# cloneofsimo/paint-with-words-sd

Hardware: NVIDIA H100
Metric: unet_steps_per_sec_512sq_cfg (higher is better)
Workload: dtype f16

## Files before the change

paint_with_words_sd_b200/csrc/attn_tc.cuh:

```cuda
#pragma once
#include "mma_sm90.cuh"
#include "pww_common.cuh"
#include "xattn_core.cuh"
#include "xattn_tc.cuh"

namespace pww {
namespace fa {

constexpr int kThreads = core::kThreads;
constexpr int kBM = core::kBM;
constexpr int kBN = 64;

template <int D>
struct Cfg {
  using T_ = core::Tile<D>;
  static constexpr uint32_t KVBYTES = kBN * T_::LD * 2;
  static constexpr uint32_t OFF_KV = T_::QBYTES;
  static constexpr uint32_t SMEM = T_::QBYTES + 2 * 2 * KVBYTES;
  static_assert(SMEM <= 232448, "shared memory budget");
};

struct Params {
  const __half* q;
  const __half* k;
  const __half* v;
  __half* out;
  int B, H, N;
  int64_t bs, rs;
  int64_t o_bs, o_rs;
  float scale;
};

template <int D>
__global__ void __launch_bounds__(kThreads) attn_fwd_kernel(const Params p) {
  using C = core::Tile<D>;
  using CF = Cfg<D>;
  extern __shared__ __align__(128) unsigned char smem[];
  const uint32_t smem0 = ptx::smem_u32(smem);
  const int warp = threadIdx.x >> 5, lane = threadIdx.x & 31;
  const int qtiles = (p.N + kBM - 1) / kBM;
  const int bh = blockIdx.x / qtiles, qt = blockIdx.x - bh * qtiles;
  const int b = bh / p.H, h = bh - b * p.H;
  const int row_base = qt * kBM;
  const __half* qb = p.q + (int64_t)b * p.bs + h * D;
  const __half* kb = p.k + (int64_t)b * p.bs + h * D;
  const __half* vb = p.v + (int64_t)b * p.bs + h * D;
  const int ntiles = (p.N + kBN - 1) / kBN;
  auto issue_kv = [&](int j) {
    const uint32_t st = smem0 + CF::OFF_KV + (j & 1) * 2 * CF::KVBYTES;
    const int rows = p.N - j * kBN < kBN ? p.N - j * kBN : kBN;
    core::load_rows<D>(st, kb + (int64_t)j * kBN * p.rs, p.rs, kBN, rows);
    core::load_rows<D>(st + CF::KVBYTES, vb + (int64_t)j * kBN * p.rs, p.rs, kBN, rows);
    ptx::cp_async_commit();
  };
  {
    const int rows = p.N - row_base < kBM ? p.N - row_base : kBM;
    core::load_rows<D>(smem0, qb + (int64_t)row_base * p.rs, p.rs, kBM, rows);
  }
  issue_kv(0);
  uint32_t qa[C::KS][4];
  float o[C::NT][4];
#pragma unroll
  for (int j = 0; j < C::NT; ++j) o[j][0] = o[j][1] = o[j][2] = o[j][3] = 0.f;
  float m0 = -INFINITY, m1 = -INFINITY, l0 = 0.f, l1 = 0.f;
  const float sl2 = p.scale * 1.4426950408889634f;
  const uint32_t qs = smem0 + (uint32_t)(warp * 16 * C::LD) * 2u;
#pragma unroll 1
  for (int jt = 0; jt < ntiles; ++jt) {
    if (jt + 1 < ntiles) {
      issue_kv(jt + 1);
      ptx::cp_async_wait<1>();
    } else {
      ptx::cp_async_wait<0>();
    }
    __syncthreads();
    if (jt == 0) {
#pragma unroll
      for (int kk = 0; kk < C::KS; ++kk)
        ptx::ldsm_x4(qs + (uint32_t)((lane & 15) * C::LD + kk * 16 + (lane >> 4) * 8) * 2u, qa[kk][0], qa[kk][1], qa[kk][2], qa[kk][3]);
    }
    const uint32_t ks = smem0 + CF::OFF_KV + (jt & 1) * 2 * CF::KVBYTES, vs = ks + CF::KVBYTES;
    float s[8][4];
#pragma unroll
    for (int j = 0; j < 8; ++j) s[j][0] = s[j][1] = s[j][2] = s[j][3] = 0.f;
#pragma unroll
    for (int kk = 0; kk < C::KS; ++kk) {
#pragma unroll
      for (int jp = 0; jp < 4; ++jp) {
        const int t = 16 * jp + (lane & 7) + ((lane >> 4) << 3), d = kk * 16 + ((lane >> 3) & 1) * 8;
        uint32_t b0, b1, b2, b3;
        ptx::ldsm_x4(ks + (uint32_t)(t * C::LD + d) * 2u, b0, b1, b2, b3);
        ptx::mma16816(s[2 * jp], qa[kk], b0, b1);
        ptx::mma16816(s[2 * jp + 1], qa[kk], b2, b3);
      }
    }
    const int valid = p.N - jt * kBN;
    float t0 = -INFINITY, t1 = -INFINITY;
#pragma unroll
    for (int j = 0; j < 8; ++j)
#pragma unroll
      for (int e = 0; e < 4; ++e) {
        if (core::tok(j, e, lane) >= valid) s[j][e] = -INFINITY;
        if (e < 2) t0 = fmaxf(t0, s[j][e]); else t1 = fmaxf(t1, s[j][e]);
      }
    t0 = fmaxf(t0, __shfl_xor_sync(0xffffffffu, t0, 1));
    t0 = fmaxf(t0, __shfl_xor_sync(0xffffffffu, t0, 2));
    t1 = fmaxf(t1, __shfl_xor_sync(0xffffffffu, t1, 1));
    t1 = fmaxf(t1, __shfl_xor_sync(0xffffffffu, t1, 2));
    const float mn0 = fmaxf(m0, t0), mn1 = fmaxf(m1, t1);
    const float a0 = ptx::ex2((m0 - mn0) * sl2), a1 = ptx::ex2((m1 - mn1) * sl2);
    m0 = mn0; m1 = mn1;
    const float n0 = -mn0 * sl2, n1 = -mn1 * sl2;
    uint32_t pa[4][4];
    float r0 = 0.f, r1 = 0.f;
#pragma unroll
    for (int j = 0; j < 8; ++j) {
      const uint32_t p01 = ptx::pack_h2(ptx::ex2(fmaf(s[j][0], sl2, n0)), ptx::ex2(fmaf(s[j][1], sl2, n0)));
      const uint32_t p23 = ptx::pack_h2(ptx::ex2(fmaf(s[j][2], sl2, n1)), ptx::ex2(fmaf(s[j][3], sl2, n1)));
      const float2 f01 = ptx::unpack_h2(p01), f23 = ptx::unpack_h2(p23);
      r0 += f01.x + f01.y;
      r1 += f23.x + f23.y;
      pa[j >> 1][(j & 1) * 2] = p01;
      pa[j >> 1][(j & 1) * 2 + 1] = p23;
    }
    l0 = l0 * a0 + r0;
    l1 = l1 * a1 + r1;
#pragma unroll
    for (int j = 0; j < C::NT; ++j) {
      o[j][0] *= a0; o[j][1] *= a0; o[j][2] *= a1; o[j][3] *= a1;
    }
#pragma unroll
    for (int kk = 0; kk < 4; ++kk) {
      const int t = 16 * kk + (lane & 7) + ((lane >> 3) & 1) * 8;
#pragma unroll
      for (int jp = 0; jp < C::NT / 2; ++jp) {
        uint32_t b0, b1, b2, b3;
        ptx::ldsm_x4_t(vs + (uint32_t)(t * C::LD + 16 * jp + (lane >> 4) * 8) * 2u, b0, b1, b2, b3);
        ptx::mma16816(o[2 * jp], pa[kk], b0, b1);
        ptx::mma16816(o[2 * jp + 1], pa[kk], b2, b3);
      }
      if constexpr (C::NT & 1) {
        uint32_t b0, b1;
        ptx::ldsm_x2_t(vs + (uint32_t)(t * C::LD + 8 * (C::NT - 1)) * 2u, b0, b1);
        ptx::mma16816(o[C::NT - 1], pa[kk], b0, b1);
      }
    }
    __syncthreads();
  }
  l0 += __shfl_xor_sync(0xffffffffu, l0, 1);
  l0 += __shfl_xor_sync(0xffffffffu, l0, 2);
  l1 += __shfl_xor_sync(0xffffffffu, l1, 1);
  l1 += __shfl_xor_sync(0xffffffffu, l1, 2);
  const float i0 = 1.f / l0, i1 = 1.f / l1;
#pragma unroll
  for (int j = 0; j < C::NT; ++j) {
    o[j][0] *= i0; o[j][1] *= i0; o[j][2] *= i1; o[j][3] *= i1;
  }
  core::warp_store<D>(o, smem + warp * 16 * C::LD * 2, lane, p.out + (int64_t)b * p.o_bs + h * D, p.o_rs,
                      row_base + warp * 16, p.N);
}

template <int D>
cudaError_t launch(const void* q, const void* k, const void* v, void* out, int B, int H, int N, int64_t bs, int64_t rs,
                   int64_t o_bs, int64_t o_rs, float scale, cudaStream_t s) {
  using CF = Cfg<D>;
  Params p;
  p.q = (const __half*)q; p.k = (const __half*)k; p.v = (const __half*)v; p.out = (__half*)out;
  p.B = B; p.H = H; p.N = N; p.bs = bs; p.rs = rs; p.o_bs = o_bs; p.o_rs = o_rs; p.scale = scale;
  static bool attr_set[tc::kMaxDevices] = {false};
  if (!attr_set[tc::cur_device()]) {
    cudaError_t e = cudaFuncSetAttribute(attn_fwd_kernel<D>, cudaFuncAttributeMaxDynamicSharedMemorySize, CF::SMEM);
    if (e != cudaSuccess) return e;
    attr_set[tc::cur_device()] = true;
  }
  const long long grid = (long long)B * H * ((N + kBM - 1) / kBM);
  if (grid > 0x7fffffffLL) return cudaErrorInvalidConfiguration;
  attn_fwd_kernel<D><<<(unsigned)grid, kThreads, CF::SMEM, s>>>(p);
  return cudaGetLastError();
}

}
}
```

paint_with_words_sd_b200/csrc/mma_sm90.cuh:

```cuda
#pragma once
#include <cuda_fp16.h>
#include <cuda_runtime.h>
#include <stdint.h>

namespace pww {
namespace ptx {

__device__ __forceinline__ uint32_t smem_u32(const void* p) { return (uint32_t)__cvta_generic_to_shared(p); }

__device__ __forceinline__ void cp_async16(uint32_t dst, const void* src, uint32_t src_bytes) {
  asm volatile("cp.async.cg.shared.global [%0], [%1], 16, %2;" ::"r"(dst), "l"(src), "r"(src_bytes) : "memory");
}
__device__ __forceinline__ void cp_async_commit() { asm volatile("cp.async.commit_group;" ::: "memory"); }
template <int N>
__device__ __forceinline__ void cp_async_wait() { asm volatile("cp.async.wait_group %0;" ::"n"(N) : "memory"); }

__device__ __forceinline__ void ldsm_x4(uint32_t addr, uint32_t& r0, uint32_t& r1, uint32_t& r2, uint32_t& r3) {
  asm volatile("ldmatrix.sync.aligned.m8n8.x4.shared.b16 {%0, %1, %2, %3}, [%4];"
               : "=r"(r0), "=r"(r1), "=r"(r2), "=r"(r3) : "r"(addr));
}
__device__ __forceinline__ void ldsm_x4_t(uint32_t addr, uint32_t& r0, uint32_t& r1, uint32_t& r2, uint32_t& r3) {
  asm volatile("ldmatrix.sync.aligned.m8n8.x4.trans.shared.b16 {%0, %1, %2, %3}, [%4];"
               : "=r"(r0), "=r"(r1), "=r"(r2), "=r"(r3) : "r"(addr));
}
__device__ __forceinline__ void ldsm_x2_t(uint32_t addr, uint32_t& r0, uint32_t& r1) {
  asm volatile("ldmatrix.sync.aligned.m8n8.x2.trans.shared.b16 {%0, %1}, [%2];" : "=r"(r0), "=r"(r1) : "r"(addr));
}

__device__ __forceinline__ void mma16816(float* c, const uint32_t* a, uint32_t b0, uint32_t b1) {
  asm volatile(
      "mma.sync.aligned.m16n8k16.row.col.f32.f16.f16.f32 {%0, %1, %2, %3}, {%4, %5, %6, %7}, {%8, %9}, "
      "{%0, %1, %2, %3};"
      : "+f"(c[0]), "+f"(c[1]), "+f"(c[2]), "+f"(c[3])
      : "r"(a[0]), "r"(a[1]), "r"(a[2]), "r"(a[3]), "r"(b0), "r"(b1));
}

__device__ __forceinline__ float ex2(float x) {
  float y;
  asm("ex2.approx.ftz.f32 %0, %1;" : "=f"(y) : "f"(x));
  return y;
}
__device__ __forceinline__ uint32_t pack_h2(float lo, float hi) {
  const __half2 h = __floats2half2_rn(lo, hi);
  return *reinterpret_cast<const uint32_t*>(&h);
}
__device__ __forceinline__ float2 unpack_h2(uint32_t v) { return __half22float2(*reinterpret_cast<const __half2*>(&v)); }
__device__ __forceinline__ unsigned long long ld_acquire_gpu_u64(const unsigned long long* p) {
  unsigned long long v;
  asm volatile("ld.acquire.gpu.global.u64 %0, [%1];" : "=l"(v) : "l"(p) : "memory");
  return v;
}

}
}
```

Before: 145.0.

## Rewrite self-attention kernel as warp-specialized TMA plus WGMMA pipeline

Replaces the cp.async and mma.sync flash-attention kernel with a Hopper-style design. A producer warp issues TMA loads of Q/K/V into 128B-swizzled shared memory through a three-stage mbarrier ring. Two consumer warpgroups run QK^T and PV as asynchronous wgmma, interleaving the next tile's QK with the previous tile's PV behind ping-pong named barriers. Row sums come from an extra wgmma against a ones matrix rather than shuffles. It targets tensor-core throughput and load latency, at the cost of much more complex synchronization, one CTA per SM, and host-side tensor map encoding on every launch.

```diff
diff --git a/paint_with_words_sd_b200/csrc/attn_tc.cuh b/paint_with_words_sd_b200/csrc/attn_tc.cuh
--- a/paint_with_words_sd_b200/csrc/attn_tc.cuh
+++ b/paint_with_words_sd_b200/csrc/attn_tc.cuh
@@ -1,163 +1,269 @@
 #pragma once
+#include <cudaTypedefs.h>
+
 #include "mma_sm90.cuh"
 #include "pww_common.cuh"
-#include "xattn_core.cuh"
 #include "xattn_tc.cuh"
 
 namespace pww {
 namespace fa {
 
-constexpr int kThreads = core::kThreads;
-constexpr int kBM = core::kBM;
-constexpr int kBN = 64;
+constexpr int kWgRows = 64;
+constexpr int kConsumerWarps = 8;
+constexpr int kThreads = (kConsumerWarps + 1) * 32;
+constexpr int kBM = 2 * kWgRows;
 
 template <int D>
 struct Cfg {
-  using T_ = core::Tile<D>;
-  static constexpr uint32_t KVBYTES = kBN * T_::LD * 2;
-  static constexpr uint32_t OFF_KV = T_::QBYTES;
-  static constexpr uint32_t SMEM = T_::QBYTES + 2 * 2 * KVBYTES;
-  static_assert(SMEM <= 232448, "shared memory budget");
+  static_assert(D == 40 || D == 64 || D == 80 || D == 160, "head dims of SD1.5 (40 / 80 / 160) and SD2.x (64)");
+  static constexpr int SLABS = (D + 63) / 64;
+  static constexpr int KS = (D + 15) / 16;
+  static constexpr int NT = D / 8;
+  static constexpr int BN = D == 160 ? 64 : 128;
+  static constexpr int STAGES = 3;
+  static constexpr uint32_t QBYTES = kWgRows * SLABS * 128;
+  static constexpr uint32_t KVBYTES = BN * SLABS * 128;
+  static constexpr uint32_t OFF_KV = 2 * QBYTES;
+  static constexpr uint32_t OFF_ONES = OFF_KV + STAGES * 2 * KVBYTES;
+  static constexpr uint32_t OFF_BAR = OFF_ONES + 1024;
+  static constexpr uint32_t SMEM = OFF_BAR + (1 + 2 * STAGES) * 8 + 1024;
+  static_assert(SMEM <= 232448, "shared memory budget (227 KiB per CTA)");
 };
 
 struct Params {
-  const __half* q;
-  const __half* k;
-  const __half* v;
+  CUtensorMap tq, tk, tv;
   __half* out;
-  int B, H, N;
-  int64_t bs, rs;
+  int H, N;
+  int bmul;
   int64_t o_bs, o_rs;
   float scale;
 };
 
 template <int D>
-__global__ void __launch_bounds__(kThreads) attn_fwd_kernel(const Params p) {
-  using C = core::Tile<D>;
-  using CF = Cfg<D>;
-  extern __shared__ __align__(128) unsigned char smem[];
-  const uint32_t smem0 = ptx::smem_u32(smem);
-  const int warp = threadIdx.x >> 5, lane = threadIdx.x & 31;
+__global__ void __launch_bounds__(kThreads, 1) attn_fwd_kernel(const __grid_constant__ Params p) {
+  using C = Cfg<D>;
+  extern __shared__ unsigned char smem_raw[];
+  const uint32_t smem0 = (ptx::smem_u32(smem_raw) + 1023u) & ~1023u;
+  const uint32_t bar_q = smem0 + C::OFF_BAR, bar_full = bar_q + 8, bar_empty = bar_full + 8 * C::STAGES;
+  const int warp = __shfl_sync(0xffffffffu, threadIdx.x >> 5, 0), lane = threadIdx.x & 31;
   const int qtiles = (p.N + kBM - 1) / kBM;
   const int bh = blockIdx.x / qtiles, qt = blockIdx.x - bh * qtiles;
   const int b = bh / p.H, h = bh - b * p.H;
   const int row_base = qt * kBM;
-  const __half* qb = p.q + (int64_t)b * p.bs + h * D;
-  const __half* kb = p.k + (int64_t)b * p.bs + h * D;
-  const __half* vb = p.v + (int64_t)b * p.bs + h * D;
-  const int ntiles = (p.N + kBN - 1) / kBN;
-  auto issue_kv = [&](int j) {
-    const uint32_t st = smem0 + CF::OFF_KV + (j & 1) * 2 * CF::KVBYTES;
-    const int rows = p.N - j * kBN < kBN ? p.N - j * kBN : kBN;
-    core::load_rows<D>(st, kb + (int64_t)j * kBN * p.rs, p.rs, kBN, rows);
-    core::load_rows<D>(st + CF::KVBYTES, vb + (int64_t)j * kBN * p.rs, p.rs, kBN, rows);
-    ptx::cp_async_commit();
-  };
-  {
-    const int rows = p.N - row_base < kBM ? p.N - row_base : kBM;
-    core::load_rows<D>(smem0, qb + (int64_t)row_base * p.rs, p.rs, kBM, rows);
-  }
-  issue_kv(0);
-  uint32_t qa[C::KS][4];
+  const int ntiles = (p.N + C::BN - 1) / C::BN;
+  for (int i = threadIdx.x; i < 1024 / 16; i += blockDim.x)
+    *reinterpret_cast<uint4*>(smem_raw + (smem0 - ptx::smem_u32(smem_raw)) + C::OFF_ONES + 16 * i) =
+        make_uint4(0x3c003c00u, 0x3c003c00u, 0x3c003c00u, 0x3c003c00u);
+  ptx::fence_proxy_async();
+  if (threadIdx.x == 0) {
+    ptx::mbar_init(bar_q, 1);
+    for (int s = 0; s < C::STAGES; ++s) {
+      ptx::mbar_init(bar_full + 8 * s, 1);
+      ptx::mbar_init(bar_empty + 8 * s, kConsumerWarps);
+    }
+    ptx::mbar_fence_init();
+  }
+  __syncthreads();
+
+  if (warp == kConsumerWarps) {
+    if (lane == 0) {
+      const int bc = b * p.bmul;
+      ptx::tma_prefetch_desc(&p.tq);
+      ptx::tma_prefetch_desc(&p.tk);
+      ptx::tma_prefetch_desc(&p.tv);
+      ptx::mbar_arrive_expect_tx(bar_q, 2 * C::QBYTES);
+#pragma unroll
+      for (int c = 0; c < C::SLABS; ++c) {
+        ptx::tma_load_4d(smem0 + c * kWgRows * 128, &p.tq, bar_q, 64 * c, row_base, h, bc);
+        ptx::tma_load_4d(smem0 + C::QBYTES + c * kWgRows * 128, &p.tq, bar_q, 64 * c, row_base + kWgRows, h, bc);
+      }
+#pragma unroll 1
+      for (int j = 0; j < ntiles; ++j) {
+        const int s = j % C::STAGES, use = j / C::STAGES;
+        if (use > 0) ptx::mbar_wait(bar_empty + 8 * s, (use - 1) & 1);
+        const uint32_t ks = smem0 + C::OFF_KV + s * 2 * C::KVBYTES;
+        ptx::mbar_arrive_expect_tx(bar_full + 8 * s, 2 * C::KVBYTES);
+#pragma unroll
+        for (int c = 0; c < C::SLABS; ++c) {
+          ptx::tma_load_4d(ks + c * C::BN * 128, &p.tk, bar_full + 8 * s, 64 * c, j * C::BN, h, bc);
+          ptx::tma_load_4d(ks + C::KVBYTES + c * C::BN * 128, &p.tv, bar_full + 8 * s, 64 * c, j * C::BN, h, bc);
+        }
+      }
+    }
+    return;
+  }
+
+  const int wg = warp >> 2, wl = warp & 3;
+  const uint32_t qs = smem0 + wg * C::QBYTES;
   float o[C::NT][4];
 #pragma unroll
   for (int j = 0; j < C::NT; ++j) o[j][0] = o[j][1] = o[j][2] = o[j][3] = 0.f;
-  float m0 = -INFINITY, m1 = -INFINITY, l0 = 0.f, l1 = 0.f;
+  float lsum[4] = {0.f, 0.f, 0.f, 0.f};
+  const uint64_t ones_desc = ptx::wgmma_desc_sw128(smem0 + C::OFF_ONES, 16, 1024);
+  float m0 = -INFINITY, m1 = -INFINITY;
   const float sl2 = p.scale * 1.4426950408889634f;
-  const uint32_t qs = smem0 + (uint32_t)(warp * 16 * C::LD) * 2u;
-#pragma unroll 1
-  for (int jt = 0; jt < ntiles; ++jt) {
-    if (jt + 1 < ntiles) {
-      issue_kv(jt + 1);
-      ptx::cp_async_wait<1>();
-    } else {
-      ptx::cp_async_wait<0>();
-    }
-    __syncthreads();
-    if (jt == 0) {
-#pragma unroll
-      for (int kk = 0; kk < C::KS; ++kk)
-        ptx::ldsm_x4(qs + (uint32_t)((lane & 15) * C::LD + kk * 16 + (lane >> 4) * 8) * 2u, qa[kk][0], qa[kk][1], qa[kk][2], qa[kk][3]);
-    }
-    const uint32_t ks = smem0 + CF::OFF_KV + (jt & 1) * 2 * CF::KVBYTES, vs = ks + CF::KVBYTES;
-    float s[8][4];
-#pragma unroll
-    for (int j = 0; j < 8; ++j) s[j][0] = s[j][1] = s[j][2] = s[j][3] = 0.f;
-#pragma unroll
-    for (int kk = 0; kk < C::KS; ++kk) {
-#pragma unroll
-      for (int jp = 0; jp < 4; ++jp) {
-        const int t = 16 * jp + (lane & 7) + ((lane >> 4) << 3), d = kk * 16 + ((lane >> 3) & 1) * 8;
-        uint32_t b0, b1, b2, b3;
-        ptx::ldsm_x4(ks + (uint32_t)(t * C::LD + d) * 2u, b0, b1, b2, b3);
-        ptx::mma16816(s[2 * jp], qa[kk], b0, b1);
-        ptx::mma16816(s[2 * jp + 1], qa[kk], b2, b3);
-      }
-    }
-    const int valid = p.N - jt * kBN;
+  float sc[C::BN / 8][4];
+  using PTile = uint32_t[C::BN / 16][4];
+  auto stage_of = [&](int jt) { return smem0 + C::OFF_KV + (jt % C::STAGES) * 2 * C::KVBYTES; };
+  auto wait_full = [&](int jt) { ptx::mbar_wait(bar_full + 8 * (jt % C::STAGES), (jt / C::STAGES) & 1); };
+  auto issue_qk = [&](int jt) {
+    const uint32_t ks = stage_of(jt);
+#pragma unroll
+    for (int kk = 0; kk < C::KS; ++kk)
+      ptx::wgmma_ss<C::BN>(&sc[0][0], ptx::wgmma_desc_sw128(qs + (kk >> 2) * kWgRows * 128 + (kk & 3) * 32, 16, 1024),
+                           ptx::wgmma_desc_sw128(ks + (kk >> 2) * C::BN * 128 + (kk & 3) * 32, 16, 1024), kk);
+    ptx::wgmma_commit();
+  };
+  auto issue_pv = [&](int jt, const PTile& pa) {
+    const uint32_t vs = stage_of(jt) + C::KVBYTES;
+#pragma unroll
+    for (int kk = 0; kk < C::BN / 16; ++kk) {
+      ptx::wgmma_rs<D>(&o[0][0], pa[kk], ptx::wgmma_desc_sw128(vs + kk * 16 * 128, C::BN * 128, 1024));
+      ptx::wgmma_rs_n8_kmajor(lsum, pa[kk], ones_desc);
+    }
+    ptx::wgmma_commit();
+  };
+  auto pv_done = [&](int jt, PTile& pa) {
+#pragma unroll
+    for (int j = 0; j < C::NT; ++j)
+#pragma unroll
+      for (int e = 0; e < 4; ++e) ptx::fence_operand(o[j][e]);
+#pragma unroll
+    for (int e = 0; e < 4; ++e) ptx::fence_operand(lsum[e]);
+#pragma unroll
+    for (int j = 0; j < C::BN / 16; ++j)
+#pragma unroll
+      for (int e = 0; e < 4; ++e) ptx::fence_operand(pa[j][e]);
+    __syncwarp();
+    if (lane == 0) ptx::mbar_arrive(bar_empty + 8 * (jt % C::STAGES));
+  };
+  float a0 = 0.f, a1 = 0.f;
+  auto softmax = [&](int jt, PTile& pn) {
+#pragma unroll
+    for (int j = 0; j < C::BN / 8; ++j)
+#pragma unroll
+      for (int e = 0; e < 4; ++e) ptx::fence_operand(sc[j][e]);
+    if (jt == ntiles - 1) {
+      const int valid = p.N - jt * C::BN;
+#pragma unroll
+      for (int j = 0; j < C::BN / 8; ++j)
+#pragma unroll
+        for (int e = 0; e < 4; ++e)
+          if (8 * j + 2 * (lane & 3) + (e & 1) >= valid) sc[j][e] = -INFINITY;
+    }
     float t0 = -INFINITY, t1 = -INFINITY;
 #pragma unroll
-    for (int j = 0; j < 8; ++j)
-#pragma unroll
-      for (int e = 0; e < 4; ++e) {
-        if (core::tok(j, e, lane) >= valid) s[j][e] = -INFINITY;
-        if (e < 2) t0 = fmaxf(t0, s[j][e]); else t1 = fmaxf(t1, s[j][e]);
-      }
+    for (int j = 0; j < C::BN / 8; ++j) {
+      t0 = fmaxf(t0, fmaxf(sc[j][0], sc[j][1]));
+      t1 = fmaxf(t1, fmaxf(sc[j][2], sc[j][3]));
+    }
     t0 = fmaxf(t0, __shfl_xor_sync(0xffffffffu, t0, 1));
     t0 = fmaxf(t0, __shfl_xor_sync(0xffffffffu, t0, 2));
     t1 = fmaxf(t1, __shfl_xor_sync(0xffffffffu, t1, 1));
     t1 = fmaxf(t1, __shfl_xor_sync(0xffffffffu, t1, 2));
     const float mn0 = fmaxf(m0, t0), mn1 = fmaxf(m1, t1);
-    const float a0 = ptx::ex2((m0 - mn0) * sl2), a1 = ptx::ex2((m1 - mn1) * sl2);
+    a0 = ptx::ex2((m0 - mn0) * sl2); a1 = ptx::ex2((m1 - mn1) * sl2);
     m0 = mn0; m1 = mn1;
     const float n0 = -mn0 * sl2, n1 = -mn1 * sl2;
-    uint32_t pa[4][4];
-    float r0 = 0.f, r1 = 0.f;
-#pragma unroll
-    for (int j = 0; j < 8; ++j) {
-      const uint32_t p01 = ptx::pack_h2(ptx::ex2(fmaf(s[j][0], sl2, n0)), ptx::ex2(fmaf(s[j][1], sl2, n0)));
-      const uint32_t p23 = ptx::pack_h2(ptx::ex2(fmaf(s[j][2], sl2, n1)), ptx::ex2(fmaf(s[j][3], sl2, n1)));
-      const float2 f01 = ptx::unpack_h2(p01), f23 = ptx::unpack_h2(p23);
-      r0 += f01.x + f01.y;
-      r1 += f23.x + f23.y;
-      pa[j >> 1][(j & 1) * 2] = p01;
-      pa[j >> 1][(j & 1) * 2 + 1] = p23;
-    }
-    l0 = l0 * a0 + r0;
-    l1 = l1 * a1 + r1;
+#pragma unroll
+    for (int j = 0; j < C::BN / 8; ++j) {
+      pn[j >> 1][(j & 1) * 2] = ptx::pack_h2(ptx::ex2(fmaf(sc[j][0], sl2, n0)), ptx::ex2(fmaf(sc[j][1], sl2, n0)));
+      pn[j >> 1][(j & 1) * 2 + 1] = ptx::pack_h2(ptx::ex2(fmaf(sc[j][2], sl2, n1)), ptx::ex2(fmaf(sc[j][3], sl2, n1)));
+    }
+  };
+  auto rescale_o = [&]() {
 #pragma unroll
     for (int j = 0; j < C::NT; ++j) {
       o[j][0] *= a0; o[j][1] *= a0; o[j][2] *= a1; o[j][3] *= a1;
     }
-#pragma unroll
-    for (int kk = 0; kk < 4; ++kk) {
-      const int t = 16 * kk + (lane & 7) + ((lane >> 3) & 1) * 8;
-#pragma unroll
-      for (int jp = 0; jp < C::NT / 2; ++jp) {
-        uint32_t b0, b1, b2, b3;
-        ptx::ldsm_x4_t(vs + (uint32_t)(t * C::LD + 16 * jp + (lane >> 4) * 8) * 2u, b0, b1, b2, b3);
-        ptx::mma16816(o[2 * jp], pa[kk], b0, b1);
-        ptx::mma16816(o[2 * jp + 1], pa[kk], b2, b3);
-      }
-      if constexpr (C::NT & 1) {
-        uint32_t b0, b1;
-        ptx::ldsm_x2_t(vs + (uint32_t)(t * C::LD + 8 * (C::NT - 1)) * 2u, b0, b1);
-        ptx::mma16816(o[C::NT - 1], pa[kk], b0, b1);
-      }
-    }
-    __syncthreads();
-  }
-  l0 += __shfl_xor_sync(0xffffffffu, l0, 1);
-  l0 += __shfl_xor_sync(0xffffffffu, l0, 2);
-  l1 += __shfl_xor_sync(0xffffffffu, l1, 1);
-  l1 += __shfl_xor_sync(0xffffffffu, l1, 2);
-  const float i0 = 1.f / l0, i1 = 1.f / l1;
+    lsum[0] *= a0; lsum[1] *= a0; lsum[2] *= a1; lsum[3] *= a1;
+  };
+  constexpr int kTurn = kConsumerWarps * 32;
+  auto turn_begin = [&]() {
+    if (wg == 0) ptx::bar_sync<1>(kTurn); else ptx::bar_sync<2>(kTurn);
+  };
+  auto turn_end = [&](bool last) {
+    if (wg == 0) ptx::bar_arrive<2>(kTurn); else if (!last) ptx::bar_arrive<1>(kTurn);
+  };
+  if (wg == 1) ptx::bar_arrive<1>(kTurn);
+  ptx::mbar_wait(bar_q, 0);
+  wait_full(0);
+  turn_begin();
+  ptx::wgmma_fence();
+  issue_qk(0);
+  turn_end(false);
+  ptx::wgmma_wait<0>();
+  auto step = [&](int jt, PTile& pp, PTile& pn) {
+    wait_full(jt);
+    rescale_o();
+    turn_begin();
+    ptx::wgmma_fence();
+    issue_qk(jt);
+    issue_pv(jt - 1, pp);
+    turn_end(false);
+    ptx::wgmma_wait<1>();
+    softmax(jt, pn);
+    ptx::wgmma_wait<0>();
+    pv_done(jt - 1, pp);
+  };
+  auto finish = [&](PTile& pp) {
+    rescale_o();
+    turn_begin();
+    ptx::wgmma_fence();
+    issue_pv(ntiles - 1, pp);
+    turn_end(true);
+    ptx::wgmma_wait<0>();
+    pv_done(ntiles - 1, pp);
+  };
+  PTile pa, pb;
+  softmax(0, pa);
+  int jt = 1;
+#pragma unroll 1
+  for (; jt + 1 < ntiles; jt += 2) {
+    step(jt, pa, pb);
+    step(jt + 1, pb, pa);
+  }
+  if (jt < ntiles) {
+    step(jt, pa, pb);
+#pragma unroll
+    for (int j = 0; j < C::BN / 16; ++j)
+#pragma unroll
+      for (int e = 0; e < 4; ++e) pa[j][e] = pb[j][e];
+  }
+  finish(pa);
+  const float i0 = 1.f / lsum[0], i1 = 1.f / lsum[2];
+  const int row = row_base + wg * kWgRows + wl * 16 + (lane >> 2);
+  __half* ob = p.out + (int64_t)b * p.o_bs + (int64_t)row * p.o_rs + h * D + 2 * (lane & 3);
 #pragma unroll
   for (int j = 0; j < C::NT; ++j) {
-    o[j][0] *= i0; o[j][1] *= i0; o[j][2] *= i1; o[j][3] *= i1;
-  }
-  core::warp_store<D>(o, smem + warp * 16 * C::LD * 2, lane, p.out + (int64_t)b * p.o_bs + h * D, p.o_rs,
-                      row_base + warp * 16, p.N);
+    if (row < p.N) *reinterpret_cast<uint32_t*>(ob + 8 * j) = ptx::pack_h2(o[j][0] * i0, o[j][1] * i0);
+    if (row + 8 < p.N) *reinterpret_cast<uint32_t*>(ob + 8 * p.o_rs + 8 * j) = ptx::pack_h2(o[j][2] * i1, o[j][3] * i1);
+  }
+}
+
+inline PFN_cuTensorMapEncodeTiled_v12000 tensor_map_encoder() {
+  static PFN_cuTensorMapEncodeTiled_v12000 fn = nullptr;
+  if (!fn) {
+    void* f = nullptr;
+    cudaDriverEntryPointQueryResult q;
+    if (cudaGetDriverEntryPoint("cuTensorMapEncodeTiled", &f, cudaEnableDefault, &q) == cudaSuccess &&
+        q == cudaDriverEntryPointSuccess)
+      fn = (PFN_cuTensorMapEncodeTiled_v12000)f;
+  }
+  return fn;
+}
+
+template <int D>
+bool make_tensor_map(CUtensorMap* m, const void* base, int rows, int B, int H, int N, int64_t bs, int64_t rs) {
+  const auto encode = tensor_map_encoder();
+  if (!encode || bs < 0) return false;
+  const cuuint64_t dims[4] = {D, (cuuint64_t)N, (cuuint64_t)H, bs == 0 ? 1 : (cuuint64_t)B};
+  const cuuint64_t strides[3] = {(cuuint64_t)rs * 2, D * 2, bs == 0 ? 16 : (cuuint64_t)bs * 2};
+  const cuuint32_t box[4] = {64, (cuuint32_t)rows, 1, 1};
+  const cuuint32_t estr[4] = {1, 1, 1, 1};
+  return encode(m, CU_TENSOR_MAP_DATA_TYPE_FLOAT16, 4, const_cast<void*>(base), dims, strides, box, estr,
+                CU_TENSOR_MAP_INTERLEAVE_NONE, CU_TENSOR_MAP_SWIZZLE_128B, CU_TENSOR_MAP_L2_PROMOTION_L2_128B,
+                CU_TENSOR_MAP_FLOAT_OOB_FILL_NONE) == CUDA_SUCCESS;
 }
 
 template <int D>
@@ -165,8 +271,11 @@
                    int64_t o_bs, int64_t o_rs, float scale, cudaStream_t s) {
   using CF = Cfg<D>;
   Params p;
-  p.q = (const __half*)q; p.k = (const __half*)k; p.v = (const __half*)v; p.out = (__half*)out;
-  p.B = B; p.H = H; p.N = N; p.bs = bs; p.rs = rs; p.o_bs = o_bs; p.o_rs = o_rs; p.scale = scale;
+  if (!make_tensor_map<D>(&p.tq, q, kWgRows, B, H, N, bs, rs) || !make_tensor_map<D>(&p.tk, k, CF::BN, B, H, N, bs, rs) ||
+      !make_tensor_map<D>(&p.tv, v, CF::BN, B, H, N, bs, rs))
+    return cudaErrorInvalidValue;
+  p.out = (__half*)out;
+  p.H = H; p.N = N; p.bmul = bs == 0 ? 0 : 1; p.o_bs = o_bs; p.o_rs = o_rs; p.scale = scale;
   static bool attr_set[tc::kMaxDevices] = {false};
   if (!attr_set[tc::cur_device()]) {
     cudaError_t e = cudaFuncSetAttribute(attn_fwd_kernel<D>, cudaFuncAttributeMaxDynamicSharedMemorySize, CF::SMEM);
diff --git a/paint_with_words_sd_b200/csrc/mma_sm90.cuh b/paint_with_words_sd_b200/csrc/mma_sm90.cuh
--- a/paint_with_words_sd_b200/csrc/mma_sm90.cuh
+++ b/paint_with_words_sd_b200/csrc/mma_sm90.cuh
@@ -51,5 +51,115 @@
   return v;
 }
 
+
+__device__ __forceinline__ void mbar_init(uint32_t bar, uint32_t count) {
+  asm volatile("mbarrier.init.shared::cta.b64 [%0], %1;" ::"r"(bar), "r"(count) : "memory");
+}
+__device__ __forceinline__ void mbar_fence_init() { asm volatile("fence.mbarrier_init.release.cluster;" ::: "memory"); }
+__device__ __forceinline__ void mbar_arrive(uint32_t bar) {
+  asm volatile("mbarrier.arrive.shared::cta.b64 _, [%0];" ::"r"(bar) : "memory");
+}
+__device__ __forceinline__ void mbar_arrive_expect_tx(uint32_t bar, uint32_t bytes) {
+  asm volatile("mbarrier.arrive.expect_tx.shared::cta.b64 _, [%0], %1;" ::"r"(bar), "r"(bytes) : "memory");
+}
+__device__ __forceinline__ void mbar_wait(uint32_t bar, uint32_t parity) {
+  asm volatile(
+      "{\n.reg .pred done;\nWAIT_%=:\n"
+      "mbarrier.try_wait.parity.shared::cta.b64 done, [%0], %1;\n"
+      "@!done bra WAIT_%=;\n}\n" ::"r"(bar), "r"(parity) : "memory");
+}
+
+template <int ID>
+__device__ __forceinline__ void bar_sync(int threads) {
+  asm volatile("bar.sync %0, %1;" ::"n"(ID), "r"(threads) : "memory");
+}
+template <int ID>
+__device__ __forceinline__ void bar_arrive(int threads) {
+  asm volatile("bar.arrive %0, %1;" ::"n"(ID), "r"(threads) : "memory");
+}
+
+__device__ __forceinline__ void tma_load_4d(uint32_t dst, const void* tmap, uint32_t bar, int c0, int c1, int c2, int c3) {
+  asm volatile(
+      "cp.async.bulk.tensor.4d.shared::cluster.global.tile.mbarrier::complete_tx::bytes [%0], [%1, {%3, %4, %5, %6}], [%2];"
+      ::"r"(dst), "l"(tmap), "r"(bar), "r"(c0), "r"(c1), "r"(c2), "r"(c3) : "memory");
+}
+__device__ __forceinline__ void tma_prefetch_desc(const void* tmap) {
+  asm volatile("prefetch.tensormap [%0];" ::"l"(tmap) : "memory");
+}
+
+__device__ __forceinline__ uint64_t wgmma_desc_sw128(uint32_t addr, uint32_t lbo, uint32_t sbo) {
+  return (uint64_t)((addr >> 4) & 0x3fff) | ((uint64_t)((lbo >> 4) & 0x3fff) << 16) |
+         ((uint64_t)((sbo >> 4) & 0x3fff) << 32) | (1ull << 62);
+}
+__device__ __forceinline__ void wgmma_fence() { asm volatile("wgmma.fence.sync.aligned;" ::: "memory"); }
+__device__ __forceinline__ void wgmma_commit() { asm volatile("wgmma.commit_group.sync.aligned;" ::: "memory"); }
+template <int N>
+__device__ __forceinline__ void wgmma_wait() { asm volatile("wgmma.wait_group.sync.aligned %0;" ::"n"(N) : "memory"); }
+__device__ __forceinline__ void fence_operand(float& r) { asm volatile("" : "+f"(r)::"memory"); }
+__device__ __forceinline__ void fence_operand(uint32_t& r) { asm volatile("" : "+r"(r)::"memory"); }
+__device__ __forceinline__ void fence_proxy_async() { asm volatile("fence.proxy.async.shared::cta;" ::: "memory"); }
+
+template <int N>
+__device__ __forceinline__ void wgmma_ss(float* d, uint64_t da, uint64_t db, int acc);
+template <int N>
+__device__ __forceinline__ void wgmma_rs(float* d, const uint32_t* a, uint64_t db);
+template <>
+__device__ __forceinline__ void wgmma_ss<64>(float* d, uint64_t da, uint64_t db, int acc) {
+  asm volatile(
+      "{\n.reg .pred p;\nsetp.ne.b32 p, %34, 0;\n"
+      "wgmma.mma_async.sync.aligned.m64n64k16.f32.f16.f16 {%0, %1, %2, %3, %4, %5, %6, %7, %8, %9, %10, %11, %12, %13, %14, %15, %16, %17, %18, %19, %20, %21, %22, %23, %24, %25, %26, %27, %28, %29, %30, %31}, %32, %33, p, 1, 1, 0, 0;\n}\n"
+      : "+f"(d[0]), "+f"(d[1]), "+f"(d[2]), "+f"(d[3]), "+f"(d[4]), "+f"(d[5]), "+f"(d[6]), "+f"(d[7]), "+f"(d[8]), "+f"(d[9]), "+f"(d[10]), "+f"(d[11]), "+f"(d[12]), "+f"(d[13]), "+f"(d[14]), "+f"(d[15]), "+f"(d[16]), "+f"(d[17]), "+f"(d[18]), "+f"(d[19]), "+f"(d[20]), "+f"(d[21]), "+f"(d[22]), "+f"(d[23]), "+f"(d[24]), "+f"(d[25]), "+f"(d[26]), "+f"(d[27]), "+f"(d[28]), "+f"(d[29]), "+f"(d[30]), "+f"(d[31])
+      : "l"(da), "l"(db), "r"(acc));
+}
+template <>
+__device__ __forceinline__ void wgmma_ss<128>(float* d, uint64_t da, uint64_t db, int acc) {
+  asm volatile(
+      "{\n.reg .pred p;\nsetp.ne.b32 p, %66, 0;\n"
+      "wgmma.mma_async.sync.aligned.m64n128k16.f32.f16.f16 {%0, %1, %2, %3, %4, %5, %6, %7, %8, %9, %10, %11, %12, %13, %14, %15, %16, %17, %18, %19, %20, %21, %22, %23, %24, %25, %26, %27, %28, %29, %30, %31, %32, %33, %34, %35, %36, %37, %38, %39, %40, %41, %42, %43, %44, %45, %46, %47, %48, %49, %50, %51, %52, %53, %54, %55, %56, %57, %58, %59, %60, %61, %62, %63}, %64, %65, p, 1, 1, 0, 0;\n}\n"
+      : "+f"(d[0]), "+f"(d[1]), "+f"(d[2]), "+f"(d[3]), "+f"(d[4]), "+f"(d[5]), "+f"(d[6]), "+f"(d[7]), "+f"(d[8]), "+f"(d[9]), "+f"(d[10]), "+f"(d[11]), "+f"(d[12]), "+f"(d[13]), "+f"(d[14]), "+f"(d[15]), "+f"(d[16]), "+f"(d[17]), "+f"(d[18]), "+f"(d[19]), "+f"(d[20]), "+f"(d[21]), "+f"(d[22]), "+f"(d[23]), "+f"(d[24]), "+f"(d[25]), "+f"(d[26]), "+f"(d[27]), "+f"(d[28]), "+f"(d[29]), "+f"(d[30]), "+f"(d[31]), "+f"(d[32]), "+f"(d[33]), "+f"(d[34]), "+f"(d[35]), "+f"(d[36]), "+f"(d[37]), "+f"(d[38]), "+f"(d[39]), "+f"(d[40]), "+f"(d[41]), "+f"(d[42]), "+f"(d[43]), "+f"(d[44]), "+f"(d[45]), "+f"(d[46]), "+f"(d[47]), "+f"(d[48]), "+f"(d[49]), "+f"(d[50]), "+f"(d[51]), "+f"(d[52]), "+f"(d[53]), "+f"(d[54]), "+f"(d[55]), "+f"(d[56]), "+f"(d[57]), "+f"(d[58]), "+f"(d[59]), "+f"(d[60]), "+f"(d[61]), "+f"(d[62]), "+f"(d[63])
+      : "l"(da), "l"(db), "r"(acc));
+}
+template <>
+__device__ __forceinline__ void wgmma_rs<40>(float* d, const uint32_t* a, uint64_t db) {
+  asm volatile(
+      "{\n.reg .pred p;\nsetp.ne.b32 p, %25, 0;\n"
+      "wgmma.mma_async.sync.aligned.m64n40k16.f32.f16.f16 {%0, %1, %2, %3, %4, %5, %6, %7, %8, %9, %10, %11, %12, %13, %14, %15, %16, %17, %18, %19}, {%20, %21, %22, %23}, %24, p, 1, 1, 1;\n}\n"
+      : "+f"(d[0]), "+f"(d[1]), "+f"(d[2]), "+f"(d[3]), "+f"(d[4]), "+f"(d[5]), "+f"(d[6]), "+f"(d[7]), "+f"(d[8]), "+f"(d[9]), "+f"(d[10]), "+f"(d[11]), "+f"(d[12]), "+f"(d[13]), "+f"(d[14]), "+f"(d[15]), "+f"(d[16]), "+f"(d[17]), "+f"(d[18]), "+f"(d[19])
+      : "r"(a[0]), "r"(a[1]), "r"(a[2]), "r"(a[3]), "l"(db), "r"(1));
+}
+template <>
+__device__ __forceinline__ void wgmma_rs<64>(float* d, const uint32_t* a, uint64_t db) {
+  asm volatile(
+      "{\n.reg .pred p;\nsetp.ne.b32 p, %37, 0;\n"
+      "wgmma.mma_async.sync.aligned.m64n64k16.f32.f16.f16 {%0, %1, %2, %3, %4, %5, %6, %7, %8, %9, %10, %11, %12, %13, %14, %15, %16, %17, %18, %19, %20, %21, %22, %23, %24, %25, %26, %27, %28, %29, %30, %31}, {%32, %33, %34, %35}, %36, p, 1, 1, 1;\n}\n"
+      : "+f"(d[0]), "+f"(d[1]), "+f"(d[2]), "+f"(d[3]), "+f"(d[4]), "+f"(d[5]), "+f"(d[6]), "+f"(d[7]), "+f"(d[8]), "+f"(d[9]), "+f"(d[10]), "+f"(d[11]), "+f"(d[12]), "+f"(d[13]), "+f"(d[14]), "+f"(d[15]), "+f"(d[16]), "+f"(d[17]), "+f"(d[18]), "+f"(d[19]), "+f"(d[20]), "+f"(d[21]), "+f"(d[22]), "+f"(d[23]), "+f"(d[24]), "+f"(d[25]), "+f"(d[26]), "+f"(d[27]), "+f"(d[28]), "+f"(d[29]), "+f"(d[30]), "+f"(d[31])
+      : "r"(a[0]), "r"(a[1]), "r"(a[2]), "r"(a[3]), "l"(db), "r"(1));
+}
+template <>
+__device__ __forceinline__ void wgmma_rs<80>(float* d, const uint32_t* a, uint64_t db) {
+  asm volatile(
+      "{\n.reg .pred p;\nsetp.ne.b32 p, %45, 0;\n"
+      "wgmma.mma_async.sync.aligned.m64n80k16.f32.f16.f16 {%0, %1, %2, %3, %4, %5, %6, %7, %8, %9, %10, %11, %12, %13, %14, %15, %16, %17, %18, %19, %20, %21, %22, %23, %24, %25, %26, %27, %28, %29, %30, %31, %32, %33, %34, %35, %36, %37, %38, %39}, {%40, %41, %42, %43}, %44, p, 1, 1, 1;\n}\n"
+      : "+f"(d[0]), "+f"(d[1]), "+f"(d[2]), "+f"(d[3]), "+f"(d[4]), "+f"(d[5]), "+f"(d[6]), "+f"(d[7]), "+f"(d[8]), "+f"(d[9]), "+f"(d[10]), "+f"(d[11]), "+f"(d[12]), "+f"(d[13]), "+f"(d[14]), "+f"(d[15]), "+f"(d[16]), "+f"(d[17]), "+f"(d[18]), "+f"(d[19]), "+f"(d[20]), "+f"(d[21]), "+f"(d[22]), "+f"(d[23]), "+f"(d[24]), "+f"(d[25]), "+f"(d[26]), "+f"(d[27]), "+f"(d[28]), "+f"(d[29]), "+f"(d[30]), "+f"(d[31]), "+f"(d[32]), "+f"(d[33]), "+f"(d[34]), "+f"(d[35]), "+f"(d[36]), "+f"(d[37]), "+f"(d[38]), "+f"(d[39])
+      : "r"(a[0]), "r"(a[1]), "r"(a[2]), "r"(a[3]), "l"(db), "r"(1));
+}
+template <>
+__device__ __forceinline__ void wgmma_rs<160>(float* d, const uint32_t* a, uint64_t db) {
+  asm volatile(
+      "{\n.reg .pred p;\nsetp.ne.b32 p, %85, 0;\n"
+      "wgmma.mma_async.sync.aligned.m64n160k16.f32.f16.f16 {%0, %1, %2, %3, %4, %5, %6, %7, %8, %9, %10, %11, %12, %13, %14, %15, %16, %17, %18, %19, %20, %21, %22, %23, %24, %25, %26, %27, %28, %29, %30, %31, %32, %33, %34, %35, %36, %37, %38, %39, %40, %41, %42, %43, %44, %45, %46, %47, %48, %49, %50, %51, %52, %53, %54, %55, %56, %57, %58, %59, %60, %61, %62, %63, %64, %65, %66, %67, %68, %69, %70, %71, %72, %73, %74, %75, %76, %77, %78, %79}, {%80, %81, %82, %83}, %84, p, 1, 1, 1;\n}\n"
+      : "+f"(d[0]), "+f"(d[1]), "+f"(d[2]), "+f"(d[3]), "+f"(d[4]), "+f"(d[5]), "+f"(d[6]), "+f"(d[7]), "+f"(d[8]), "+f"(d[9]), "+f"(d[10]), "+f"(d[11]), "+f"(d[12]), "+f"(d[13]), "+f"(d[14]), "+f"(d[15]), "+f"(d[16]), "+f"(d[17]), "+f"(d[18]), "+f"(d[19]), "+f"(d[20]), "+f"(d[21]), "+f"(d[22]), "+f"(d[23]), "+f"(d[24]), "+f"(d[25]), "+f"(d[26]), "+f"(d[27]), "+f"(d[28]), "+f"(d[29]), "+f"(d[30]), "+f"(d[31]), "+f"(d[32]), "+f"(d[33]), "+f"(d[34]), "+f"(d[35]), "+f"(d[36]), "+f"(d[37]), "+f"(d[38]), "+f"(d[39]), "+f"(d[40]), "+f"(d[41]), "+f"(d[42]), "+f"(d[43]), "+f"(d[44]), "+f"(d[45]), "+f"(d[46]), "+f"(d[47]), "+f"(d[48]), "+f"(d[49]), "+f"(d[50]), "+f"(d[51]), "+f"(d[52]), "+f"(d[53]), "+f"(d[54]), "+f"(d[55]), "+f"(d[56]), "+f"(d[57]), "+f"(d[58]), "+f"(d[59]), "+f"(d[60]), "+f"(d[61]), "+f"(d[62]), "+f"(d[63]), "+f"(d[64]), "+f"(d[65]), "+f"(d[66]), "+f"(d[67]), "+f"(d[68]), "+f"(d[69]), "+f"(d[70]), "+f"(d[71]), "+f"(d[72]), "+f"(d[73]), "+f"(d[74]), "+f"(d[75]), "+f"(d[76]), "+f"(d[77]), "+f"(d[78]), "+f"(d[79])
+      : "r"(a[0]), "r"(a[1]), "r"(a[2]), "r"(a[3]), "l"(db), "r"(1));
+}
+
+
+__device__ __forceinline__ void wgmma_rs_n8_kmajor(float* d, const uint32_t* a, uint64_t db) {
+  asm volatile(
+      "{\n.reg .pred p;\nsetp.ne.b32 p, %9, 0;\n"
+      "wgmma.mma_async.sync.aligned.m64n8k16.f32.f16.f16 {%0, %1, %2, %3}, {%4, %5, %6, %7}, %8, p, 1, 1, 0;\n}\n"
+      : "+f"(d[0]), "+f"(d[1]), "+f"(d[2]), "+f"(d[3])
+      : "r"(a[0]), "r"(a[1]), "r"(a[2]), "r"(a[3]), "l"(db), "r"(1));
+}
+
 }
 }
```

Result: faster. 147.0 (median of 6 runs) (+1.4%).
